# Juleszwanen/oscar_mpc_planner_mr_modification

Hardware: AMD Instinct MI355X
Metric: SQP solves/s (N=20, 8 obs, 8 guesses) at 1/2/4/8 MI355X; max |x−x_ref| (higher is better)
Workload: dtype f64

## Files before the change

__graft_entry__.py:

```python
import os
import sys

ROOT = os.path.dirname(os.path.abspath(__file__))
if ROOT not in sys.path:
    sys.path.insert(0, ROOT)


def build() -> None:
    from oscar_mpc_planner_mr_modification_amd import _build

    _build.build_lib()
    for cfg in ("C2", "C5", "C3", "JS"):
        _build.build_cpp(cfg)
    from oscar_mpc_planner_mr_modification_amd.layouts import tmpc_layout
    _build.build_instance(tmpc_layout(N=25, max_obstacles=3, name="G25"), os.path.join(_build.BUILD, "G25"))
    _build.build_stage_probe()
    sys.path.insert(0, os.path.join(ROOT, "oracle"))
    import oracle_py

    oracle_py.build()
    import oscar_mpc_planner_mr_modification_amd
    from oscar_mpc_planner_mr_modification_amd import native


def smoke() -> None:
    import numpy as np
    import torch

    sys.path.insert(0, os.path.join(ROOT, "oracle"))
    import oracle_py
    from oscar_mpc_planner_mr_modification_amd import native
    from oscar_mpc_planner_mr_modification_amd.layouts import config_layout
    from oscar_mpc_planner_mr_modification_amd.synthetic import make_batch

    assert torch.cuda.is_available(), "smoke() needs an MI355X"
    dev = torch.device("cuda:0")
    lay = config_layout("C2")
    b = make_batch(lay, 2, 8, seed=20251212)
    pr = native.problem_from_layout(lay)
    t = lambda a: torch.from_numpy(np.ascontiguousarray(a)).to(dev)
    out = native.solve_batch_device(pr, t(b.params), t(b.warm), t(b.xinit))
    torch.cuda.synchronize()
    ref = oracle_py.Oracle(lay).solve_batch(b.params, b.warm, b.xinit)
    exit_gpu = out["exit"].cpu().numpy()
    assert np.array_equal(exit_gpu, ref["status"]), (exit_gpu, ref["status"])
    ok = exit_gpu == 1
    assert ok.any()
    dx = np.abs(out["xtraj"].cpu().numpy()[ok] - ref["xtraj"][ok]).max()
    assert dx <= 1e-4, dx
    print(f"smoke ok: {len(exit_gpu)} solves, {int(ok.sum())} successful, max|x-x_ref| = {dx:.2e}")


if __name__ == "__main__":
    build()
    if len(sys.argv) > 1 and sys.argv[1] == "smoke":
        smoke()
```

oscar_mpc_planner_mr_modification_amd/_build.py:

```python
from __future__ import annotations

import os
import subprocess

PKG = os.path.dirname(os.path.abspath(__file__))
ROOT = os.path.dirname(PKG)
CSRC = os.path.join(PKG, "csrc")
INCLUDE = os.path.join(ROOT, "include")
LIB = os.path.join(PKG, "libmpcg.so")
ARCH = os.environ.get("MPCG_OFFLOAD_ARCH", "gfx950")

SOURCES = {"mpcg_kernels.hip": [], "mpcg_prepare.hip": ["-ffp-contract=off"],
           "mpcg_inst_tmpc20.hip": [], "mpcg_inst_tmpc30.hip": [], "mpcg_inst_shmpc.hip": [],
           "mpcg_inst_bicycle.hip": []}
HEADERS = ["mpcg_device.h", "mpcg_sqp.h", "mpcg_sqp_body.inc", "mpcg_prepare.h", "mpcg_bicycle.h", "mpcg_instance.h"]
FLEET_SOURCES = {"mpcg_fleet.hip": ["-ffp-contract=off"]}
FLEET_HEADERS = ["mpcg_fleet.h"]
PATH_SOURCES = {"mpcg_path.hip": ["-ffp-contract=off"]}
PATH_HEADERS = ["mpcg_path.h"]
GUIDANCE_SOURCES = {"mpcg_guidance.hip": ["-ffp-contract=off"]}
GUIDANCE_HEADERS = ["mpcg_guidance.h"]
ACTIVE_SOURCES = {"mpcg_active.hip": ["-ffp-contract=off"]}
ACTIVE_HEADERS = ["mpcg_active.h"]
HOST_SOURCES = ["host/mpcg_yaml.cpp", "host/mpcg_solver.cpp"]
HOST_HEADERS = ["mpc_planner_solver/mpcg_yaml.h", "mpc_planner_solver/mpcg_config.h", "mpc_planner_solver/state.h",
                "mpc_planner_solver/mpcg_solver_interface.h", "mpc_planner_solver/solver_interface.h"]
BUILD = os.path.join(PKG, "build")


def source_hash() -> str:
    import hashlib

    h = hashlib.sha256()
    for f in sorted(list(SOURCES) + HEADERS):
        h.update(f.encode())
        with open(os.path.join(CSRC, f), "rb") as fh:
            h.update(fh.read())
    with open(os.path.join(INCLUDE, "mpcg.h"), "rb") as fh:
        h.update(fh.read())
    h.update(repr((ARCH, sorted(SOURCES.items()))).encode())
    return h.hexdigest()


def _stale(target, deps):
    if not os.path.exists(target):
        return True
    t = os.path.getmtime(target)
    return any(os.path.getmtime(d) > t for d in deps)


def build_lib(force: bool = False, verbose: bool = False, extra_flags=(), out: str = LIB, sources=None) -> str:
    srcs = SOURCES if sources is None else {k: v for k, v in SOURCES.items() if k in sources}
    srcs = {**srcs, **FLEET_SOURCES, **PATH_SOURCES, **GUIDANCE_SOURCES, **ACTIVE_SOURCES}
    deps = [os.path.join(CSRC, s) for s in list(SOURCES) + HEADERS + list(FLEET_SOURCES) + FLEET_HEADERS +
            list(PATH_SOURCES) + PATH_HEADERS + list(GUIDANCE_SOURCES) + GUIDANCE_HEADERS +
            list(ACTIVE_SOURCES) + ACTIVE_HEADERS] + \
        [os.path.join(INCLUDE, h) for h in ("mpcg.h", "mpcg_fleet.h", "mpcg_path.h", "mpcg_guidance.h",
                                            "mpcg_active.h")] + [__file__]
    if not force and not _stale(out, deps):
        return out
    objdir = os.path.join(BUILD, "obj" + ("_" + "_".join(f.strip("-").replace("=", "") for f in extra_flags)
                                          if extra_flags else ""))
    os.makedirs(objdir, exist_ok=True)
    common = ["hipcc", f"--offload-arch={ARCH}", "-O3", "-std=c++17", "-fPIC", f"-I{INCLUDE}", f"-I{CSRC}"]
    objs, procs = [], []
    for src, flags in srcs.items():
        obj = os.path.join(objdir, src.replace(".hip", ".o"))
        cmd = common + list(flags) + list(extra_flags) + ["-c", os.path.join(CSRC, src), "-o", obj]
        if verbose:
            print(" ".join(cmd))
        procs.append(subprocess.Popen(cmd))
        objs.append(obj)
    for p in procs:
        if p.wait() != 0:
            raise subprocess.CalledProcessError(p.returncode, "hipcc")
    cmd = ["hipcc", f"--offload-arch={ARCH}", "-shared", "-fPIC", "-Wl,-soname,libmpcg.so", "-o", out + ".tmp"] + objs
    if verbose:
        print(" ".join(cmd))
    subprocess.run(cmd, check=True)
    os.replace(out + ".tmp", out)
    return out


def _hipcc_obj(src, obj, extra=()):
    cmd = ["hipcc", f"--offload-arch={ARCH}", "-O3", "-std=c++17", "-fPIC", f"-I{INCLUDE}", f"-I{CSRC}",
           *extra, "-c", src, "-o", obj]
    subprocess.run(cmd, check=True)
    return obj


def build_instance(layout, out_dir: str, force: bool = False) -> str:
    from . import codegen

    lib_mpcg = build_lib()
    os.makedirs(out_dir, exist_ok=True)
    src = os.path.join(out_dir, "mpcg_instance.hip")
    text = codegen.instance_source(layout)
    if not os.path.exists(src) or open(src).read() != text:
        with open(src, "w") as fh:
            fh.write(text)
    so = os.path.join(out_dir, f"libmpcg_inst_{layout.name}.so")
    deps = [src, lib_mpcg, os.path.join(INCLUDE, "mpcg.h")] + [os.path.join(CSRC, h) for h in HEADERS]
    if force or _stale(so, deps):
        obj = _hipcc_obj(src, os.path.join(out_dir, "mpcg_instance.o"))
        subprocess.run(["hipcc", f"--offload-arch={ARCH}", "-shared", "-fPIC", "-o", so + ".tmp", obj, f"-L{PKG}",
                        "-lmpcg", f"-Wl,-rpath,{PKG}"], check=True)
        os.replace(so + ".tmp", so)
    return so


def build_stage_probe(force: bool = False) -> str:
    src = os.path.join(ROOT, "tests", "cpp", "stage_probe.hip")
    out_dir = os.path.join(BUILD, "probe")
    so = os.path.join(out_dir, "libstage_probe.so")
    deps = [src, os.path.join(INCLUDE, "mpcg.h"), __file__] + [os.path.join(CSRC, h) for h in HEADERS]
    if force or _stale(so, deps):
        os.makedirs(out_dir, exist_ok=True)
        obj = _hipcc_obj(src, os.path.join(out_dir, "stage_probe.o"))
        subprocess.run(["hipcc", f"--offload-arch={ARCH}", "-shared", "-fPIC", "-o", so + ".tmp", obj], check=True)
        os.replace(so + ".tmp", so)
    return so


def build_cpp(config="C2", force: bool = False, verbose: bool = False) -> dict:
    from . import codegen
    from .layouts import config_layout

    lay = config_layout(config) if isinstance(config, str) else config
    lib_mpcg = build_lib()
    out = os.path.join(BUILD, lay.name)
    codegen.generate(lay, out)
    so = os.path.join(out, "libmpc_planner_solver.so")
    exe = os.path.join(out, "test_solver")
    srcs = [os.path.join(CSRC, s) for s in HOST_SOURCES] + [os.path.join(out, "mpc_planner_parameters.cpp")]
    inst = os.path.join(out, "mpcg_instance.hip")
    deps = srcs + [inst] + [os.path.join(INCLUDE, h) for h in HOST_HEADERS] + \
        [os.path.join(CSRC, h) for h in HEADERS] + [os.path.join(INCLUDE, "mpcg.h"), lib_mpcg, __file__]
    inc = [f"-I{os.path.join(out, 'include')}", f"-I{INCLUDE}"]
    if force or _stale(so, deps):
        objs = []
        for src in srcs:
            obj = os.path.join(out, os.path.basename(src).replace(".cpp", ".o"))
            cmd = ["g++", "-std=c++17", "-O2", "-fPIC", "-Wall", "-Wextra"] + inc + ["-c", src, "-o", obj]
            if verbose:
                print(" ".join(cmd))
            subprocess.run(cmd, check=True)
            objs.append(obj)
        objs.append(_hipcc_obj(inst, os.path.join(out, "mpcg_instance.o")))
        cmd = ["hipcc", f"--offload-arch={ARCH}", "-shared", "-fPIC"] + objs + \
              ["-o", so + ".tmp", f"-L{PKG}", "-lmpcg", f"-Wl,-rpath,{PKG}"]
        if verbose:
            print(" ".join(cmd))
        subprocess.run(cmd, check=True)
        os.replace(so + ".tmp", so)
    test_src = os.path.join(ROOT, "tests", "cpp", "test_solver.cpp")
    if os.path.exists(test_src) and (force or _stale(exe, [test_src, so])):
        cmd = ["g++", "-std=c++17", "-O2", "-Wall", "-Wextra"] + inc + [test_src, "-o", exe, f"-L{out}",
                                                                      "-lmpc_planner_solver", f"-L{PKG}", "-lmpcg",
                                                                      f"-Wl,-rpath,{out}:{PKG}"]
        if verbose:
            print(" ".join(cmd))
        subprocess.run(cmd, check=True)
    return {"dir": out, "lib": so, "test": exe}


if __name__ == "__main__":
    print(build_lib(force=True, verbose=True))
    print(build_cpp("C2", force=True, verbose=True))
```

oscar_mpc_planner_mr_modification_amd/csrc/mpcg_device.h:

```cpp
#pragma once
#include <hip/hip_runtime.h>

#include "mpcg.h"

namespace mpcg {

constexpr int NU = MPCG_NU;

__device__ __forceinline__ double frcp(double x) {
    double y = __builtin_amdgcn_rcp(x);
    double e = fma(-x, y, 1.0);
    y = fma(y, e, y);
    e = fma(-x, y, 1.0);
    return fma(y, e, y);
}

__device__ __forceinline__ double frsq(double x) {
    double y = __builtin_amdgcn_rsq(x);
    const double h = 0.5 * x;
    y = y * fma(-h * y, y, 1.5);
    return y * fma(-h * y, y, 1.5);
}

__device__ __forceinline__ double fsqrt_pos(double x) { return x * frsq(x); }
// ... 128 lines not shown
    const double wc = p[pr.i_w_contour], wl = p[pr.i_w_lag];
    double L = wa * a * a + ww * w * w + wv * (v - vref) * (v - vref);
    SplineJets J;
    spline_jets(pr, p, s, J);
    const double rsq = J.Dx[0] * J.Dx[0] + J.Dy[0] * J.Dy[0];
    const double ir = frsq(rsq);
    const double tx = J.Dx[0] * ir, ty = J.Dy[0] * ir;
    const double ex = x - J.Gx[0], ey = y - J.Gy[0];
    const double ec = ty * ex - tx * ey;
    const double el = tx * ex + ty * ey;
    L += wl * el * el + wc * ec * ec;
    double wcn = 0.0, dxp = 0.0, dyp = 0.0;
    if (pr.i_cons_w >= 0) {
        wcn = p[pr.i_cons_w];
        dxp = x - p[pr.i_prev_x];
        dyp = y - p[pr.i_prev_y];
        L += wcn * (dxp * dxp + dyp * dyp);
    }
    double wsl = 0.0, sl = 0.0;
    if constexpr (NX > 5) {
        wsl = p[pr.i_w_slack];
        sl = z[NU + 5];
        L += wsl * sl * sl;
    }
    if (!derivs) return L;
    const double r1 = tx * J.Dx[1] + ty * J.Dy[1];
    const double tx1 = (J.Dx[1] - tx * r1) * ir, ty1 = (J.Dy[1] - ty * r1) * ir;
    const double r2 = tx1 * J.Dx[1] + ty1 * J.Dy[1] + tx * J.Dx[2] + ty * J.Dy[2];
    const double tx2 = (J.Dx[2] - 2.0 * tx1 * r1 - tx * r2) * ir;
    const double ty2 = (J.Dy[2] - 2.0 * ty1 * r1 - ty * r2) * ir;
    const double Gx1 = J.Gx[1], Gy1 = J.Gy[1], Gx2 = J.Gx[2], Gy2 = J.Gy[2];
    const double dc[3] = {ty, -tx, ty1 * ex - tx1 * ey - ty * Gx1 + tx * Gy1};
    const double dl[3] = {tx, ty, tx1 * ex + ty1 * ey - tx * Gx1 - ty * Gy1};
    const double hc_s[3] = {ty1, -tx1, ty2 * ex - tx2 * ey - 2.0 * ty1 * Gx1 + 2.0 * tx1 * Gy1 - ty * Gx2 + tx * Gy2};
    const double hl_s[3] = {tx1, ty1, tx2 * ex + ty2 * ey - 2.0 * tx1 * Gx1 - 2.0 * ty1 * Gy1 - tx * Gx2 - ty * Gy2};
#pragma unroll
    for (int i = 0; i < NZ; ++i) {
        g[i] = 0.0;
#pragma unroll
        for (int j = 0; j < NZ; ++j) H[i][j] = 0.0;
    }
    g[0] = 2.0 * wa * a; H[0][0] = 2.0 * wa;
    g[1] = 2.0 * ww * w; H[1][1] = 2.0 * ww;
    g[5] = 2.0 * wv * (v - vref); H[5][5] = 2.0 * wv;
    constexpr int ids[3] = {2, 3, 6};
#pragma unroll
    for (int i = 0; i < 3; ++i) {
        g[ids[i]] += 2.0 * (wl * el * dl[i] + wc * ec * dc[i]);
#pragma unroll
        for (int j = 0; j < 3; ++j) {
            double hl = (i == 2) ? hl_s[j] : ((j == 2) ? hl_s[i] : 0.0);
            double hc = (i == 2) ? hc_s[j] : ((j == 2) ? hc_s[i] : 0.0);
            H[ids[i]][ids[j]] += 2.0 * (wl * (dl[i] * dl[j] + el * hl) + wc * (dc[i] * dc[j] + ec * hc));
        }
    }
    if (pr.i_cons_w >= 0) {
        g[2] += 2.0 * wcn * dxp; g[3] += 2.0 * wcn * dyp;
        H[2][2] += 2.0 * wcn; H[3][3] += 2.0 * wcn;
    }
    if constexpr (NX > 5) {
        g[NU + 5] = 2.0 * wsl * sl;
        H[NU + 5][NU + 5] = 2.0 * wsl;
    }
    return L;
}

__device__ __forceinline__ void erk_srow(const mpcg_problem& pr, double& sa, double& sv) {
    sa = 0.5 * pr.dt * pr.dt;
    sv = pr.dt;
}

template <int NX>
__device__ inline void erk_unicycle(const mpcg_problem& pr, const double z[NU + NX], const double* pi,
                                    double xn[NX], double F[NX][NU + NX], double H[NU + NX][NU + NX]) {
    constexpr int NZ = NU + NX;
    const double a = z[0], w = z[1], psi = z[4], v = z[5];
    const int ns = pr.rk_steps;
    const double h = pr.dt / ns;
    double sx = 0.0, sy = 0.0, ss = 0.0;
    double jx[4] = {0, 0, 0, 0}, jy[4] = {0, 0, 0, 0}, js[4] = {0, 0, 0, 0};
    double hq[4][4];
#pragma unroll
    for (int i = 0; i < 4; ++i)
#pragma unroll
        for (int j = 0; j < 4; ++j) hq[i][j] = 0.0;
    const double pix = pi ? pi[0] : 0.0, piy = pi ? pi[1] : 0.0;
    double cpsi, spsi;
    sincos(psi, &spsi, &cpsi);
    for (int st = 0; st < ns; ++st) {
#pragma unroll
        for (int q = 0; q < 4; ++q) {
            const double cq = (q == 0) ? 0.0 : ((q == 3) ? 1.0 : 0.5);
            const double bq = ((q == 0 || q == 3) ? 1.0 : 2.0) * h / 6.0;
            const double tau = (st + cq) * h;
            double sw, cw;
            sincos(tau * w, &sw, &cw);
            const double ce = cpsi * cw - spsi * sw;
            const double se = spsi * cw + cpsi * sw;
            const double ve = v + tau * a;
            sx += bq * ve * ce;
            sy += bq * ve * se;
            ss += bq * ve;
            const double dcx_p = -ve * se, dcx_v = ce;
            const double dcy_p = ve * ce, dcy_v = se;
            jx[0] += bq * dcx_v * tau; jx[1] += bq * dcx_p * tau; jx[2] += bq * dcx_p; jx[3] += bq * dcx_v;
            jy[0] += bq * dcy_v * tau; jy[1] += bq * dcy_p * tau; jy[2] += bq * dcy_p; jy[3] += bq * dcy_v;
            if (pi) {
                const double hpp = bq * (-pix * ve * ce - piy * ve * se);
                const double hpv = bq * (-pix * se + piy * ce);
                const double rp[4] = {0.0, tau, 1.0, 0.0};
                const double rv[4] = {tau, 0.0, 0.0, 1.0};
#pragma unroll
                for (int i = 0; i < 4; ++i)
#pragma unroll
                    for (int j = 0; j < 4; ++j)
                        hq[i][j] += hpp * rp[i] * rp[j] + hpv * (rp[i] * rv[j] + rv[i] * rp[j]);
            }
        }
    }
    erk_srow(pr, js[0], js[3]);
    const double T = pr.dt;
    xn[0] = z[2] + sx;
    xn[1] = z[3] + sy;
    xn[2] = psi + T * w;
    xn[3] = v + T * a;
    xn[4] = z[6] + ss;
#pragma unroll
    for (int i = 0; i < NX; ++i)
#pragma unroll
        for (int j = 0; j < NZ; ++j) F[i][j] = 0.0;
    constexpr int zi[4] = {0, 1, 4, 5};
#pragma unroll
    for (int j = 0; j < 4; ++j) {
        F[0][zi[j]] = jx[j];
        F[1][zi[j]] = jy[j];
        F[4][zi[j]] = js[j];
    }
    F[0][2] = 1.0; F[1][3] = 1.0; F[4][6] = 1.0;
    F[2][1] = T; F[2][4] = 1.0;
    F[3][0] = T; F[3][5] = 1.0;
#pragma unroll
    for (int i = 5; i < NX; ++i) {
        xn[i] = z[NU + i];
        F[i][NU + i] = 1.0;
    }
    if (pi) {
#pragma unroll
        for (int i = 0; i < 4; ++i)
#pragma unroll
            for (int j = 0; j < 4; ++j) H[zi[i]][zi[j]] += hq[i][j];
    }
}

template <int NZ, int NA = NZ>
__device__ inline void mirror(double A[NZ][NZ], double eps, double dia_extra = 0.0) {
    double V[NA][NA];
#pragma unroll
    for (int i = 0; i < NA; ++i)
#pragma unroll
        for (int j = 0; j < NA; ++j) {
            V[i][j] = (i == j) ? 1.0 : 0.0;
            if (j > i) A[i][j] = 0.5 * (A[i][j] + A[j][i]);
        }
    for (int sweep = 0; sweep < 50; ++sweep) {
        double off = 0.0, dia = 0.0;
#pragma unroll
        for (int i = 0; i < NA; ++i) {
            dia += A[i][i] * A[i][i];
            if (i == NA - 1) dia += dia_extra;
#pragma unroll
            for (int j = i + 1; j < NA; ++j) off += A[i][j] * A[i][j];
        }
        if (off <= 1e-32 * dia || off < 1e-300) break;
#pragma unroll
        for (int p = 0; p < NA - 1; ++p)
#pragma unroll
            for (int q = p + 1; q < NA; ++q) {
                const double apq = A[p][q];
                if (fabs(apq) >= 1e-300) {
                    const double theta = 0.5 * (A[q][q] - A[p][p]) * frcp(apq);
                    const double at = fabs(theta);
                    double t = at < 1e150 ? frcp(at + fsqrt_pos(fma(at, at, 1.0))) : 0.5 * frcp(at);
                    t = theta >= 0.0 ? t : -t;
                    const double c = frsq(fma(t, t, 1.0)), sn = t * c;
                    const double tau = sn * frcp(1.0 + c);
                    A[p][p] -= t * apq;
                    A[q][q] += t * apq;
                    A[p][q] = 0.0;
#pragma unroll
                    for (int r = 0; r < NA; ++r) {
                        if (r == p || r == q) continue;
                        double& arp = r < p ? A[r][p] : A[p][r];
                        double& arq = r < q ? A[r][q] : A[q][r];
                        const double g = arp, h = arq;
                        arp = g - sn * fma(g, tau, h);
                        arq = h + sn * fma(-h, tau, g);
                    }
#pragma unroll
                    for (int r = 0; r < NA; ++r) {
                        const double g = V[r][p], h = V[r][q];
                        V[r][p] = g - sn * fma(g, tau, h);
                        V[r][q] = h + sn * fma(-h, tau, g);
                    }
                }
            }
    }
    double d[NA];
#pragma unroll
    for (int i = 0; i < NA; ++i) {
        double di = A[i][i];
        d[i] = (di >= -eps && di <= eps) ? eps : fabs(di);
    }
#pragma unroll
    for (int i = 0; i < NA; ++i)
#pragma unroll
        for (int j = i; j < NA; ++j) {
            double acc = 0.0;
#pragma unroll
            for (int k = 0; k < NA; ++k) acc += V[i][k] * d[k] * V[j][k];
            A[i][j] = acc;
            A[j][i] = acc;
        }
}

}
```

oscar_mpc_planner_mr_modification_amd/csrc/mpcg_sqp.h:

```cpp
#pragma once
#include <hip/hip_runtime.h>

#include <type_traits>

#include "mpcg.h"
#include "mpcg_bicycle.h"
#include "mpcg_device.h"

namespace mpcg {

enum { AC_SUCCESS = 0, AC_NAN = 1, AC_MAXITER = 2, AC_MINSTEP = 3, AC_QP_FAILURE = 4 };

__host__ __device__ constexpr int imax(int a, int b) { return a > b ? a : b; }
__host__ __device__ constexpr int sym(int i, int j) { return i >= j ? i * (i + 1) / 2 + j : j * (j + 1) / 2 + i; }
__host__ __device__ constexpr int cpk(int n, int a, int c) { return c * n - c * (c - 1) / 2 + (a - c); }

__host__ __device__ constexpr int lds_b64_cycles(int s, int off, int parts) {
    int total = 0;
    for (int half = 0; half < 2; ++half) {
        int dw[64] = {};
        int n = 0;
        for (int l = 32 * half; l < 32 * half + 32; ++l) {
            const int a = 2 * (s * (l / parts) + off * (l % parts));
            for (int h = 0; h < 2; ++h) {
                bool seen = false;
                for (int i = 0; i < n; ++i) seen = seen || dw[i] == a + h;
                if (!seen) dw[n++] = a + h;
            }
        }
        int worst = 0;
        for (int b = 0; b < 64; ++b) {
            int c = 0;
            for (int i = 0; i < n; ++i) c += (dw[i] % 64) == b;
            worst = c > worst ? c : worst;
        }
        total += worst;
    }
    return total;
}
__host__ __device__ constexpr int lds_stride(int base, int off, int parts, int step, int maxpad) {
    int best = base, bc = lds_b64_cycles(base, off, parts);
    for (int s = base + step; s <= base + maxpad; s += step) {
        const int c = lds_b64_cycles(s, off, parts);
        if (c < bc) { bc = c; best = s; }
    }
    return best;
}

template <int N_, int NL_, int NE_, int NS_ = 0, int NX_ = 5, int MODEL_ = 0>
struct Cfg {
    static constexpr int N = N_, NL = NL_, NE = NE_, NS = NS_, MODEL = MODEL_;
    static constexpr int NU = MODEL_ == 1 ? 3 : 2;
    static constexpr int NX = NX_, NZ = NU + NX_;
    static_assert(MODEL_ == 1 ? NX == 6 : (NX == 5 || NX == 6), "unicycle (+ slack state) or bicycle");
    static constexpr int IX = NU, IY = NU + 1, IPSI = NU + 2;
    static constexpr bool HAS_SLACK = MODEL_ == 1 || NX > 5;
    static constexpr int ZSL = MODEL_ == 1 ? 2 : NU + 5;
    static constexpr int NLO = NU * (NU - 1) / 2, NLC = NU == 2 ? 4 : NLO + NU;
    __host__ __device__ static constexpr int lo_idx(int i, int j) { return i * (i - 1) / 2 + j; }
    static constexpr int NH = NL + NE + NS;
    static constexpr int NTRI = NZ * (NZ + 1) / 2;
    static constexpr int NPT = NX * (NX + 1) / 2;
    static constexpr int NPTP = (MODEL_ != 1 && (64 / (N_ + 1)) >= 3) ? NPT + (NPT & 1) : NPT;
    static constexpr int NB = (HAS_SLACK && NS > 0) ? 4 : 3;
    static constexpr int NBT = NB * (NB + 1) / 2;
    static constexpr int NDH = NZ + NBT + 1;
#ifndef MPCG_PARTS_BIKE
#define MPCG_PARTS_BIKE 2
#endif
    static constexpr int PARTS_MAX = (64 / (N + 1)) >= 3 ? 3 : 2;
    static constexpr int PARTS = MODEL_ == 1 ? (MPCG_PARTS_BIKE < PARTS_MAX ? MPCG_PARTS_BIKE : PARTS_MAX) : PARTS_MAX;
    static_assert((N + 1) * PARTS <= 64, "horizon too long for one wavefront");
    static_assert(NTRI <= 64, "stage block larger than a wavefront");
    static constexpr bool QUEUE = MODEL_ == 0 && PARTS_MAX == 3;
    static constexpr int BVS = (NZ + PARTS - 1) / PARTS;
    static constexpr int HS = (NH + PARTS - 1) / PARTS;
    static constexpr int SLOTS = 2 * BVS + HS;
#ifdef MPCG_STORE_IT_ANY
    static constexpr bool STORE_IT_ANY = true;
#else
    static constexpr bool STORE_IT_ANY = false;
#endif
    static constexpr bool STORE_IT = SLOTS <= (PARTS == 3 ? 13 : STORE_IT_ANY ? 12 : 0);
    static constexpr int NBOX = 2 * NU + 2 * NX;
    static constexpr bool LIN_PARAMS = NS > 0 || N >= 30;
    static constexpr int DGC = LIN_PARAMS ? 2 : 3;
    static constexpr int NHS = LIN_PARAMS ? (NE > 0 ? NE : 1) : NH;
    static constexpr bool RELOAD_PARAMS = NS > 0 || N >= 30;
    static constexpr int M_TOTAL = 2 * NU + (N - 1) * (NBOX + NH);
    __host__ __device__ static constexpr int blk(int v) {
        return (v >= IX && v <= IPSI) ? v - IX : ((NB == 4 && v == ZSL) ? 3 : -1);
    }
    __host__ __device__ static constexpr int bvar(int b) { return b < 3 ? IX + b : ZSL; }
    static constexpr bool COMPACT = MODEL_ == 1;
    static constexpr bool FCONST = MODEL_ == 0 && N_ >= 30;
    static constexpr int NFR = COMPACT ? 4 : (FCONST ? 2 : NX), NFC = COMPACT ? NZ - 1 : NZ;
    static constexpr int NHP = COMPACT ? (NZ - 1) * NZ / 2 + 1 : NTRI;
    static constexpr bool CHAIN_SPLIT = !COMPACT;
    static constexpr bool PAIR_WANTED = FCONST && NE_ <= 8;
    static constexpr bool PAIR_CHAINS = PAIR_WANTED && CHAIN_SPLIT && (N_ + 1) / 2 * NX_ * NX_ <= (N_ + 1) * NDH &&
                                        (N_ + 1) / 2 * NX_ <= 128;
    static constexpr bool FAC_FLAT = !COMPACT;
    static constexpr bool REC_FLAT = CHAIN_SPLIT && PARTS == 3;
#ifndef MPCG_RES_CARRY
#define MPCG_RES_CARRY 1
#endif
    static constexpr bool RES_CARRY = MPCG_RES_CARRY > 0 && MODEL_ == 0 && PARTS == 3 && NX_ == 5;
    static constexpr int QPM_ROWS = 2 * SLOTS * 64;
    static constexpr int QPM = QPM_ROWS + (N + 1) * NZ + N * NX;
    __host__ __device__ static constexpr double slack_coef(int hh) { return (NB == 4 && hh >= NL + NE) ? -1.0 : 0.0; }
};

template <class C, bool LEAN = C::COMPACT, bool GFH = false, int PAD = 0>
struct Lds {
    static constexpr int N = C::N, NX = C::NX, NZ = C::NZ;
    static constexpr int DGS =
        PAD ? lds_stride(C::NHS * C::DGC, C::DGC, C::PARTS, C::DGC % 2 == 0 ? 2 : 1, 3) : C::NHS * C::DGC;
    static constexpr int HDS = PAD ? lds_stride(C::NHS, 1, C::PARTS, 1, 3) : C::NHS;
    static constexpr int PS = PAD == 0   ? C::NPTP
                              : PAD == 2 ? lds_stride(C::NPT + (C::NPT & 1), 0, C::PARTS, 2, 4)
                                         : lds_stride(C::NPTP, 0, C::PARTS, C::NPTP == C::NPT ? 1 : 2, 4);
    double z[N + 1][NZ];
    double H[GFH ? 1 : N + 1][C::NHP];
    double g[N + 1][NZ];
    double F[GFH ? 1 : N][C::NFR][C::NFC];
    double Fst[GFH && !C::COMPACT ? C::NFR : 1][C::NFC];
    double Hst[GFH && !C::COMPACT ? C::NHP : 1];
    double b[N][NX];
    double dH[N + 1][C::NDH];
    double q[N + 1][NZ];
    double dz[N + 1][NZ];
    double ddz[N + 1][NZ];
    double pi_nlp[N][NX];
    double piq[N][NX];
    double pin[LEAN ? 1 : N][NX];
    double rdyn[LEAN ? 1 : N][NX];
    alignas(16) double P[N + 1][PS];
    double Lc[N][C::NLC];
    double Y[N][C::NU][NX];
    double bx[N + 1][NZ];
    double Dg[N][DGS];
    double hd[N][HDS];
    double disc[C::LIN_PARAMS ? N : 1][4];
    double Msc[128];
    double xinit[NX];
    int flag;
};

constexpr size_t LDS_QUARTER = 160 * 1024 / 4;
template <class C>
__host__ __device__ constexpr bool lds_lean() {
    return C::COMPACT || (sizeof(Lds<C, false>) > LDS_QUARTER && sizeof(Lds<C, true>) <= LDS_QUARTER);
}
template <class C>
__host__ __device__ constexpr bool lds_gfh() {
    return sizeof(Lds<C, lds_lean<C>(), false>) > LDS_QUARTER && sizeof(Lds<C, lds_lean<C>(), true>) <= LDS_QUARTER;
}
template <class C>
__host__ __device__ constexpr int lds_pad() {
    constexpr bool P_ALIGN = !C::COMPACT;
    return P_ALIGN && sizeof(Lds<C, lds_lean<C>(), lds_gfh<C>(), 2>) <= LDS_QUARTER ? 2
           : sizeof(Lds<C, lds_lean<C>(), lds_gfh<C>(), 1>) <= LDS_QUARTER         ? 1
                                                                                   : 0;
}
template <class C>
using LdsOf = Lds<C, lds_lean<C>(), lds_gfh<C>(), lds_pad<C>()>;
template <class C>
__host__ __device__ constexpr size_t gfh_doubles() {
    return lds_gfh<C>() ? (size_t)C::N * C::NFR * C::NFC + (size_t)(C::N + 1) * C::NHP : 0;
}
template <class C>
__host__ __device__ constexpr size_t itref_doubles() {
    return 2 * (size_t)(C::N + 1) * C::NZ + (size_t)C::N * C::NX;
}
template <class C>
__host__ __device__ constexpr size_t ws_doubles() {
    return gfh_doubles<C>() + itref_doubles<C>();
}

#ifdef MPCG_STAMPS
#define MPCG_NSTAMP 24
#define STAMP_DECL unsigned long long st_acc_[MPCG_NSTAMP] = {}, st_t0_ = 0, st_l_ = 0;
#define STAMP_BEGIN() do { __syncthreads(); st_t0_ = __builtin_amdgcn_s_memtime(); st_l_ = st_t0_; } while (0)
#define STAMP_END(i) do { __syncthreads(); st_acc_[i] += __builtin_amdgcn_s_memtime() - st_t0_; } while (0)
#define STAMP_LAP(i) do { const unsigned long long t_ = __builtin_amdgcn_s_memtime(); st_acc_[i] += t_ - st_l_; st_l_ = t_; } while (0)
#define STAMP_STORE(ptr, sol) \
    do { if ((ptr) && threadIdx.x == 0) for (int i_ = 0; i_ < MPCG_NSTAMP; ++i_) (ptr)[(size_t)(sol) * MPCG_NSTAMP + i_] = st_acc_[i_]; } while (0)
#elif defined(MPCG_MARKERS)
#define STAMP_DECL
#define STAMP_BEGIN() asm volatile("; @@begin")
#define STAMP_END(i) asm volatile("; @@end " #i)
#define STAMP_LAP(i) asm volatile("; @@lap " #i)
#define STAMP_STORE(ptr, sol) do {} while (0)
#else
#define STAMP_DECL
#define STAMP_BEGIN() do {} while (0)
#define STAMP_END(i) do {} while (0)
#define STAMP_LAP(i) do {} while (0)
#define STAMP_STORE(ptr, sol) do {} while (0)
#endif

__device__ __forceinline__ void wave_sync() { __asm__ volatile("" ::: "memory"); }

typedef __attribute__((address_space(3))) double lds_double;
__device__ __forceinline__ unsigned sel_lanes(unsigned long long mask, unsigned off, unsigned on) {
    unsigned r;
    asm volatile("v_cndmask_b32_e64 %0, %1, %2, %3" : "=v"(r) : "v"(off), "v"(on), "s"(mask));
    return r;
}
__device__ __forceinline__ unsigned lds_addr(double* p) { return (unsigned)(size_t)(lds_double*)p; }
__device__ __forceinline__ void lds_store(unsigned a, double v) { *(lds_double*)(size_t)a = v; }
__device__ __forceinline__ double readlane_d(double v, int lane) {
    const int lo = __builtin_amdgcn_readlane(__double2loint(v), lane);
    const int hi = __builtin_amdgcn_readlane(__double2hiint(v), lane);
    return __hiloint2double(hi, lo);
}
template <int CTRL, int ROW_MASK = 0xF>
__device__ __forceinline__ double dpp_d(double v) {
    const int lo = __builtin_amdgcn_update_dpp(__double2loint(v), __double2loint(v), CTRL, ROW_MASK, 0xF, false);
    const int hi = __builtin_amdgcn_update_dpp(__double2hiint(v), __double2hiint(v), CTRL, ROW_MASK, 0xF, false);
    return __hiloint2double(hi, lo);
}
__device__ __forceinline__ double lane_down(double v, int p) {
    double w = dpp_d<0x130>(v);
    if (p == 2) w = dpp_d<0x130>(w);
    return w;
}
__device__ __forceinline__ double wave_max(double v) {
    v = fmax(v, dpp_d<0xB1>(v));
    v = fmax(v, dpp_d<0x4E>(v));
    v = fmax(v, dpp_d<0x141>(v));
    v = fmax(v, dpp_d<0x140>(v));
    v = fmax(v, dpp_d<0x142, 0xA>(v));
    v = fmax(v, dpp_d<0x143, 0xC>(v));
    return readlane_d(v, 63);
}
__device__ __forceinline__ double wave_sum(double v) {
    v += dpp_d<0xB1>(v);
    v += dpp_d<0x4E>(v);
    v += dpp_d<0x141>(v);
    v += dpp_d<0x140>(v);
    v += dpp_d<0x142, 0xA>(v);
    v += dpp_d<0x143, 0xC>(v);
    return readlane_d(v, 63);
}


template <int n>
__device__ __forceinline__ double chain_dot(double h, const double* G, const double* v) {
    double a = h;
#pragma unroll
    for (int j = 0; j < n; ++j) a += G[j] * v[j];
    return a;
}

template <class C>
__device__ __forceinline__ double dh_at(const double* dh, int i, int j) {
    double v = (i == j) ? dh[i] : 0.0;
    const int a = C::blk(i), c = C::blk(j);
    if (a >= 0 && c >= 0) v += dh[C::NZ + (a >= c ? cpk(C::NB, a, c) : cpk(C::NB, c, a))];
// ... 159 lines not shown
```

oscar_mpc_planner_mr_modification_amd/csrc/mpcg_sqp_body.inc:

```
    constexpr int N = C::N, PARTS = C::PARTS, NX = C::NX, NZ = C::NZ, NB = C::NB, NBT = C::NBT;
    constexpr int NU = C::NU;
    constexpr int ZS = C::ZSL;
    constexpr int X0 = C::IX, X1 = C::IY, X2 = C::IPSI;
    constexpr bool LEAN = lds_lean<C>();
    constexpr bool GFH = lds_gfh<C>();
    constexpr bool RES_SPLIT = !C::COMPACT && 2 * NB <= NZ && PARTS == 3 && NX == 5;
    constexpr int DRS = (NX + PARTS - 1) / PARTS;
    static_assert(!(RES_SPLIT && LEAN), "the split passes read the dynamics multipliers from S.pin");
    constexpr bool RES_CARRY = C::RES_CARRY && RES_SPLIT && !LEAN;
    constexpr bool CFLAG = !LEAN && !C::HAS_SLACK;
    __shared__ LdsOf<C> S;
    if (sol >= batch) return;
    if (blockDim.x != 64) {
        if (threadIdx.x == 0) io.exit_code[sol] = -1;
        return;
    }
#ifdef MPCG_LDS_POISON
    for (int e = threadIdx.x; e < (int)(sizeof(S) / 8); e += 64) ((double*)&S)[e] = __builtin_nan("");
    wave_sync();
#endif
    int lane_ = threadIdx.x;
    if constexpr (C::QUEUE) __asm__ volatile("" : "+v"(lane_));
    const int lane = lane_;
    const int k = lane / PARTS;
// ... 73 lines not shown
            return S.hd[k][hh - C::NL];
        } else {
            return S.hd[k][hh];
        }
    };
    double srow_a = 0.0, srow_v = 0.0;
    if constexpr (C::FCONST) erk_srow(pr, srow_a, srow_v);
    auto FatB = [&](const double (*Fk)[C::NFC], int m, int j) -> double {
        if constexpr (C::FCONST) {
            if (m == 2) return j == 1 ? pr.dt : (j == 4 ? 1.0 : 0.0);
            if (m == 3) return j == 0 ? pr.dt : (j == 5 ? 1.0 : 0.0);
            if (m == 4) return j == 0 ? srow_a : (j == 5 ? srow_v : (j == 6 ? 1.0 : 0.0));
            if (m >= 5) return j == NU + m ? 1.0 : 0.0;
            return Fk[m][j];
        } else if constexpr (C::COMPACT) {
            if (m == 3) return j == bike::ZV ? 1.0 : (j == bike::ZA ? pr.dt : 0.0);
            if (m == 4) return j == bike::ZDELTA ? 1.0 : (j == bike::ZW ? pr.dt : 0.0);
            if (j == ZS) return 0.0;
            return Fk[m < 3 ? m : 3][j < ZS ? j : j - 1];
        } else {
            return Fk[m][j];
        }
    };
    auto HatB = [&](const double* Hk, int i, int j) -> double {
        if constexpr (C::COMPACT) {
            if (i == ZS || j == ZS) return (i == j) ? Hk[C::NHP - 1] : 0.0;
            return Hk[sym(i < ZS ? i : i - 1, j < ZS ? j : j - 1)];
        } else {
            return Hk[sym(i, j)];
        }
    };
    auto Fat = [&](int kq, int m, int j) -> double { return FatB(Fb(kq), m, j); };
    auto Hat = [&](int kq, int i, int j) -> double { return HatB(Hb(kq), i, j); };
    auto rdyn_at = [&](int kq, int i) -> double {
        double a = S.b[kq][i] - S.dz[kq + 1][NU + i];
#pragma unroll
        for (int j = 0; j < NZ; ++j) a += Fat(kq, i, j) * S.dz[kq][j];
        return a;
    };
    auto stepped = [](double x, double a, double dx) -> double { return x + a * dx; };
    Rows<C> R;
#pragma unroll
    for (int r = 0; r < HS; ++r)
        R.nlam[r] = (lam_in && LR.h_on(r)) ? lam_in[(size_t)k * LAMS + NX + LR.hrow(r)] : 0.0;

    const double* w = io.warm + (size_t)sol * (N + 1) * NZ;
    for (int e = lane; e < (N + 1) * NZ; e += 64) (&S.z[0][0])[e] = w[e];
    for (int e = lane; e < N * NX; e += 64)
        (&S.pi_nlp[0][0])[e] = lam_in ? lam_in[(size_t)(e / NX) * LAMS + e % NX] : 0.0;
    if (lane < NX) S.xinit[lane] = io.xinit[(size_t)sol * NX + lane];
    for (int e = lane; e <= N; e += 64) S.dH[e][C::NDH - 1] = 0.0;
    const bool qp_warm = FULL && pr.qp_warm_start == 2;
    const bool sqp_mode = FULL && pr.nlp_solver == MPCG_NLP_SQP;
    bool have_qp = false;
    if (FULL && io.qp_in && !isnan(io.qp_in[(size_t)sol * C::QPM])) {
        const double* q = io.qp_in + (size_t)sol * C::QPM;
#pragma unroll
        for (int sl = 0; sl < C::SLOTS; ++sl) {
            R.t[sl] = q[(2 * sl) * 64 + lane];
            R.l[sl] = q[(2 * sl + 1) * 64 + lane];
        }
        for (int e = lane; e < (N + 1) * NZ; e += 64) (&S.dz[0][0])[e] = q[C::QPM_ROWS + e];
        for (int e = lane; e < N * NX; e += 64) (&S.piq[0][0])[e] = q[C::QPM_ROWS + (N + 1) * NZ + e];
        have_qp = true;
    }
    wave_sync();
    if (lane < NU) S.z[N][lane] = 0.0;
    wave_sync();

    constexpr bool PH = PROF == PROF_HPIPM, PRB = PROF == PROF_ROBUST;
    const bool p_move = PH ? true : PRB ? false : pr.qp_init_move != 0;
    const bool p_cond = PH ? true : PRB ? false : pr.qp_cond_pred_corr != 0;
    const int p_itref = PH ? 2 : PRB ? 0 : pr.qp_itref_corr_max;
    const bool p_sclip = PH ? false : PRB ? true : pr.qp_sigma_clip != 0;
    const bool p_maxit_first = PH ? true : PRB ? false : pr.qp_maxit_first != 0;
    const bool p_pzero = PH ? true : PRB ? false : pr.qp_pivot_zero != 0;
    const double mu_max = PH ? __builtin_inf() : pr.qp_mu_max > 0.0 ? pr.qp_mu_max : __builtin_inf(), tmin = pr.qp_t_min;
    const bool itref_on = p_itref > 0;
    int acados_status = AC_SUCCESS, qp_status = AC_SUCCESS, sqp_iter = 0, qp_total = 0, n_maxit = 0;
    double res_eq = 0.0;
    double nlp_stat = 0.0, nlp_ineq = 0.0, nlp_comp = 0.0;
    bool nlp_nonfinite = false;

    for (int it = 0; sqp_mode || it < pr.sqp_iters; ++it) {
        if constexpr (C::RELOAD_PARAMS) asm volatile("" : "+v"(pk));
        STAMP_BEGIN();
        {
            double zk[NZ];
#pragma unroll
            for (int i = 0; i < NZ; ++i) zk[i] = S.z[ks][i];
            double hb6[6] = {0, 0, 0, 0, 0, 0};
            if (k >= 1 && k < N) h_rows<C>(pr, pk, zk, LR, R.nlam, hb6, (double (*)[C::DGC])S.Dg[k], S.hd[k], S.disc[C::LIN_PARAMS ? k : 0]);
            STAMP_LAP(10);
            {
                double acc[6];
#pragma unroll
                for (int i = 0; i < 6; ++i) acc[i] = hb6[i];
#pragma unroll
                for (int p = 1; p < PARTS; ++p)
#pragma unroll
                    for (int i = 0; i < 6; ++i) acc[i] += lane_down(hb6[i], p);
#pragma unroll
                for (int i = 0; i < 6; ++i) hb6[i] = acc[i];
            }
            double resl = 0.0;
            double H[NZ][NZ];
            if (stage_lane && k < N) {
                double g[NZ], xn[NX], pi[NX];
#pragma unroll
                for (int i = 0; i < NX; ++i) pi[i] = S.pi_nlp[k][i];
                if constexpr (C::MODEL == 1) {
                    double* const Hd = Hb(k);
                    bike::discrete(pr, pk, zk, pi, xn, Fb(k), Hd);
                    STAMP_LAP(12);
                    bike::stage_cost(pr, pk, k, zk, g, H, true);
                    STAMP_LAP(11);
#pragma unroll
                    for (int i = 0; i < NZ; ++i)
#pragma unroll
                        for (int j = 0; j < NZ; ++j)
                            if (i != ZS && j != ZS) H[i][j] += Hd[sym(i < ZS ? i : i - 1, j < ZS ? j : j - 1)];
#pragma unroll
                    for (int i = 0; i < NX; ++i) {
                        const double bi = xn[i] - S.z[k + 1][NU + i];
                        S.b[k][i] = bi;
                        resl = fmax(resl, fabs(bi));
                    }
                } else {
                    double F[NX][NZ];
                    stage_cost<NX>(pr, pk, zk, g, H, true);
                    STAMP_LAP(11);
                    erk_unicycle<NX>(pr, zk, pi, xn, F, H);
                    STAMP_LAP(12);
#pragma unroll
                    for (int i = 0; i < NX; ++i) {
                        const double bi = xn[i] - S.z[k + 1][NU + i];
                        S.b[k][i] = bi;
                        resl = fmax(resl, fabs(bi));
                        if (i < C::NFR) {
#pragma unroll
                            for (int j = 0; j < NZ; ++j) Fb(k)[i][j] = F[i][j];
                        }
                    }
                }
#pragma unroll
                for (int i = 0; i < NZ; ++i) S.g[k][i] = g[i];
                H[X0][X0] += hb6[0]; H[X0][X1] += hb6[1]; H[X1][X0] += hb6[1];
                H[X0][X2] += hb6[2]; H[X2][X0] += hb6[2];
                H[X1][X1] += hb6[3]; H[X1][X2] += hb6[4]; H[X2][X1] += hb6[4];
                H[X2][X2] += hb6[5];
                STAMP_LAP(13);
                if constexpr (C::MODEL == 0 && NZ == 8) {
                    const double hs = H[NZ - 1][NZ - 1];
                    mirror<NZ, NZ - 1>(H, pr.reg_eps, hs * hs);
                    H[NZ - 1][NZ - 1] = (hs >= -pr.reg_eps && hs <= pr.reg_eps) ? pr.reg_eps : fabs(hs);
                } else if constexpr (C::MODEL == 1) {
                    double Hp[NZ][NZ];
#pragma unroll
                    for (int i = 0; i < NZ; ++i)
#pragma unroll
                        for (int j = 0; j < NZ; ++j) {
                            const int pi2 = i == NZ - 1 ? ZS : (i < ZS ? i : i + 1);
                            const int pj2 = j == NZ - 1 ? ZS : (j < ZS ? j : j + 1);
                            Hp[i][j] = H[pi2][pj2];
                        }
                    const double hs = Hp[NZ - 1][NZ - 1];
                    mirror<NZ, NZ - 1>(Hp, pr.reg_eps, hs * hs);
                    Hp[NZ - 1][NZ - 1] = (hs >= -pr.reg_eps && hs <= pr.reg_eps) ? pr.reg_eps : fabs(hs);
#pragma unroll
                    for (int i = 0; i < NZ; ++i)
#pragma unroll
                        for (int j = 0; j < NZ; ++j) {
                            const int pi2 = i == NZ - 1 ? ZS : (i < ZS ? i : i + 1);
                            const int pj2 = j == NZ - 1 ? ZS : (j < ZS ? j : j + 1);
                            H[pi2][pj2] = Hp[i][j];
                        }
                } else {
                    mirror<NZ>(H, pr.reg_eps);
                }
                STAMP_LAP(14);
                if constexpr (C::COMPACT) {
#pragma unroll
                    for (int i = 0; i < NZ; ++i)
#pragma unroll
                        for (int j = 0; j <= i; ++j)
                            if (i != ZS && j != ZS) Hb(k)[sym(i < ZS ? i : i - 1, j < ZS ? j : j - 1)] = H[i][j];
                    Hb(k)[C::NHP - 1] = H[ZS][ZS];
                } else {
#pragma unroll
                    for (int i = 0; i < NZ; ++i)
#pragma unroll
                        for (int j = 0; j <= i; ++j) Hb(k)[sym(i, j)] = H[i][j];
                }
            } else if (stage_lane && k == N) {
#pragma unroll
                for (int i = 0; i < NZ; ++i) S.g[N][i] = 0.0;
#pragma unroll
                for (int e = 0; e < C::NHP; ++e) Hb(N)[e] = 0.0;
#pragma unroll
                for (int i = NU; i < NZ; ++i) {
                    if constexpr (C::COMPACT) Hb(N)[sym(i - 1, i - 1)] = pr.reg_eps;
                    else Hb(N)[sym(i, i)] = pr.reg_eps;
                }
            }
            res_eq = wave_max(resl);
            if (lane < NX) S.dz[0][NU + lane] = S.xinit[lane] - S.z[0][NU + lane];
        }
        if constexpr (GFH) __builtin_amdgcn_fence(__ATOMIC_ACQ_REL, "workgroup");
        wave_sync();
        STAMP_END(0);

        STAMP_BEGIN();
        if (FULL && (io.stats || sqp_mode)) {
            double rh[NB];
#pragma unroll
            for (int i = 0; i < NB; ++i) rh[i] = 0.0;
            double vin = 0.0, vcp = 0.0, vst = 0.0;
            double chk = 0.0;
#pragma unroll
            for (int j = 0; j < BVS; ++j) {
                double lb = 0.0;
                if (LR.box_on(j)) {
                    const double zv = S.z[k][LR.var(j)];
                    const double gl = zv - LR.lo_at(j), gh = LR.hi_at(j) - zv;
                    const double ll = have_qp ? R.l[2 * j] : 0.0, lh = have_qp ? R.l[2 * j + 1] : 0.0;
                    chk += 0.0 * (zv + ll + lh);
                    vin = fmax(vin, -gl);
                    vin = fmax(vin, -gh);
                    vcp = fmax(vcp, fabs(ll * gl));
                    vcp = fmax(vcp, fabs(lh * gh));
                    lb = lh - ll;
                }
                if (k <= N && LR.var(j) < NZ) S.bx[k][LR.var(j)] = lb;
            }
#pragma unroll
            for (int r = 0; r < HS; ++r) {
                if (!LR.h_on(r)) continue;
                const int hh = LR.hrow(r);
                double a, bq, c;
                rowg(hh, a, bq, c);
                const double gap = rowgap(hh);
                const double lam = have_qp ? R.l[HB + r] : R.nlam[r];
                rh[0] += a * lam; rh[1] += bq * lam; rh[2] += c * lam;
                if constexpr (NB == 4) rh[3] += C::slack_coef(hh) * lam;
                vin = fmax(vin, -gap);
                vcp = fmax(vcp, fabs(lam * gap));
                chk += 0.0 * (gap + lam);
            }
            double acc[NB];
#pragma unroll
            for (int i = 0; i < NB; ++i) acc[i] = rh[i];
#pragma unroll
            for (int p = 1; p < PARTS; ++p)
#pragma unroll
                for (int i = 0; i < NB; ++i) acc[i] += lane_down(rh[i], p);
            wave_sync();
            if (stage_lane) {
                double r[NZ];
#pragma unroll
                for (int i = 0; i < NZ; ++i) r[i] = S.g[k][i] + S.bx[k][i];
#pragma unroll
                for (int i = 0; i < NB; ++i) r[C::bvar(i)] += acc[i];
                if (k < N) {
#pragma unroll
                    for (int m = 0; m < NX; ++m) {
                        const double pm = S.pi_nlp[k][m];
#pragma unroll
                        for (int i = 0; i < NZ; ++i) r[i] += Fat(k, m, i) * pm;
                    }
                }
                if (k > 0) {
#pragma unroll
                    for (int i = 0; i < NX; ++i) r[NU + i] -= S.pi_nlp[k - 1][i];
                }
#pragma unroll
                for (int i = 0; i < NZ; ++i) {
                    const bool free_var = (k == N) ? (i >= NU) : ((k == 0) ? (i < NU) : true);
                    if (free_var) vst = fmax(vst, fabs(r[i]));
                    chk += 0.0 * r[i];
                }
                if (k < N) {
#pragma unroll
                    for (int i = 0; i < NX; ++i) chk += 0.0 * S.b[k][i];
                }
            }
            nlp_stat = wave_max(vst);
            nlp_ineq = wave_max(vin);
            nlp_comp = wave_max(vcp);
            nlp_nonfinite = !(wave_sum(chk) == 0.0);
            wave_sync();
        }
        if (sqp_mode) {
            if (nlp_nonfinite) {
                acados_status = AC_NAN;
                break;
            }
            if (nlp_stat < pr.nlp_tol && res_eq < pr.nlp_tol && nlp_ineq < pr.nlp_tol && nlp_comp < pr.nlp_tol) {
                acados_status = AC_SUCCESS;
                break;
            }
            if (it >= pr.nlp_max_iter) {
                acados_status = AC_MAXITER;
                break;
            }
        }
        const bool warm_now = qp_warm && have_qp && ((sqp_mode && it > 0) || pr.qp_warm_first);
        bool hcold = false;
        if (warm_now) {
            const double thr = pr.qp_ws_thr;
#pragma unroll
            for (int sl = 0; sl < C::SLOTS; ++sl) {
                if (R.t[sl] < thr) R.t[sl] = thr;
                if (R.l[sl] < thr) R.l[sl] = thr;
                R.pr[sl] = 0.0;
            }
        } else {
        if (stage_lane) {
#pragma unroll
            for (int i = 0; i < NZ; ++i)
                if (!(k == 0 && i >= NU)) S.dz[k][i] = 0.0;
            if (k < N) {
#pragma unroll
                for (int i = 0; i < NX; ++i) S.piq[k][i] = 0.0;
            }
        }
        {
            const double thr0 = pr.qp_thr0, mu0 = pr.qp_mu0;
            const bool mv = p_move;
            auto cold = [&](int s, double gap) {
// ... 1672 lines not shown
```

Baseline: 556,500.

## Exploit block structure of stage Hessian in Jacobi eigen-regularisation

Adds a block-diagonal variant of the Jacobi eigenvalue mirror routine that skips rotations, updates and reconstruction terms coupling the two independent index blocks of the unicycle's 7x7 Hessian. A wave-wide ballot checks that the cross-block entries are exactly zero and finite on every lane, and falls back to the full routine otherwise. The intent is to cut the per-stage Jacobi sweep cost. In exchange it adds a check and a branch, and the sweep order and convergence test change, which could shift numerics slightly. It is enabled by default for PARTS==3, NX==5 model-0 configs, and a probe build target is added.

```diff
diff --git a/__graft_entry__.py b/__graft_entry__.py
--- a/__graft_entry__.py
+++ b/__graft_entry__.py
@@ -15,6 +15,7 @@
     from oscar_mpc_planner_mr_modification_amd.layouts import tmpc_layout
     _build.build_instance(tmpc_layout(N=25, max_obstacles=3, name="G25"), os.path.join(_build.BUILD, "G25"))
     _build.build_stage_probe()
+    _build.build_mirror_probe()
     sys.path.insert(0, os.path.join(ROOT, "oracle"))
     import oracle_py
 
diff --git a/oscar_mpc_planner_mr_modification_amd/_build.py b/oscar_mpc_planner_mr_modification_amd/_build.py
--- a/oscar_mpc_planner_mr_modification_amd/_build.py
+++ b/oscar_mpc_planner_mr_modification_amd/_build.py
@@ -122,6 +122,19 @@
     return so
 
 
+def build_mirror_probe(force: bool = False) -> str:
+    src = os.path.join(ROOT, "tests", "cpp", "mirror_probe.hip")
+    out_dir = os.path.join(BUILD, "probe")
+    so = os.path.join(out_dir, "libmirror_probe.so")
+    deps = [src, os.path.join(INCLUDE, "mpcg.h"), __file__, os.path.join(CSRC, "mpcg_device.h")]
+    if force or _stale(so, deps):
+        os.makedirs(out_dir, exist_ok=True)
+        obj = _hipcc_obj(src, os.path.join(out_dir, "mirror_probe.o"))
+        subprocess.run(["hipcc", f"--offload-arch={ARCH}", "-shared", "-fPIC", "-o", so + ".tmp", obj], check=True)
+        os.replace(so + ".tmp", so)
+    return so
+
+
 def build_cpp(config="C2", force: bool = False, verbose: bool = False) -> dict:
     from . import codegen
     from .layouts import config_layout
diff --git a/oscar_mpc_planner_mr_modification_amd/csrc/mpcg_device.h b/oscar_mpc_planner_mr_modification_amd/csrc/mpcg_device.h
--- a/oscar_mpc_planner_mr_modification_amd/csrc/mpcg_device.h
+++ b/oscar_mpc_planner_mr_modification_amd/csrc/mpcg_device.h
@@ -304,13 +304,17 @@
     }
 }
 
-template <int NZ, int NA = NZ>
+__host__ __device__ constexpr int mirror_blk(int i) { return (i == 2 || i == 3 || i == 6) ? 1 : 0; }
+template <int NZ, int NA = NZ, bool BLOCKS = false>
 __device__ inline void mirror(double A[NZ][NZ], double eps, double dia_extra = 0.0) {
+    static_assert(!BLOCKS || NA == 7, "the block form is the unicycle's 7 x 7 block");
+    constexpr auto in = [](int i, int j) { return !BLOCKS || mirror_blk(i) == mirror_blk(j); };
     double V[NA][NA];
 #pragma unroll
     for (int i = 0; i < NA; ++i)
 #pragma unroll
         for (int j = 0; j < NA; ++j) {
+            if (!in(i, j)) continue;
             V[i][j] = (i == j) ? 1.0 : 0.0;
             if (j > i) A[i][j] = 0.5 * (A[i][j] + A[j][i]);
         }
@@ -321,13 +325,15 @@
             dia += A[i][i] * A[i][i];
             if (i == NA - 1) dia += dia_extra;
 #pragma unroll
-            for (int j = i + 1; j < NA; ++j) off += A[i][j] * A[i][j];
+            for (int j = i + 1; j < NA; ++j)
+                if (in(i, j)) off += A[i][j] * A[i][j];
         }
         if (off <= 1e-32 * dia || off < 1e-300) break;
 #pragma unroll
         for (int p = 0; p < NA - 1; ++p)
 #pragma unroll
             for (int q = p + 1; q < NA; ++q) {
+                if (!in(p, q)) continue;
                 const double apq = A[p][q];
                 if (fabs(apq) >= 1e-300) {
                     const double theta = 0.5 * (A[q][q] - A[p][p]) * frcp(apq);
@@ -341,7 +347,7 @@
                     A[p][q] = 0.0;
 #pragma unroll
                     for (int r = 0; r < NA; ++r) {
-                        if (r == p || r == q) continue;
+                        if (r == p || r == q || !in(r, p)) continue;
                         double& arp = r < p ? A[r][p] : A[p][r];
                         double& arq = r < q ? A[r][q] : A[q][r];
                         const double g = arp, h = arq;
@@ -350,6 +356,7 @@
                     }
 #pragma unroll
                     for (int r = 0; r < NA; ++r) {
+                        if (!in(r, p)) continue;
                         const double g = V[r][p], h = V[r][q];
                         V[r][p] = g - sn * fma(g, tau, h);
                         V[r][q] = h + sn * fma(-h, tau, g);
@@ -369,10 +376,32 @@
         for (int j = i; j < NA; ++j) {
             double acc = 0.0;
 #pragma unroll
-            for (int k = 0; k < NA; ++k) acc += V[i][k] * d[k] * V[j][k];
+            for (int k = 0; k < NA; ++k)
+                if (in(i, j) && in(i, k)) acc += V[i][k] * d[k] * V[j][k];
             A[i][j] = acc;
             A[j][i] = acc;
         }
 }
 
-}
+template <int NZ>
+__device__ inline bool mirror_blocks_ok(const double A[NZ][NZ]) {
+    bool ok = true;
+#pragma unroll
+    for (int i = 0; i < 7; ++i)
+#pragma unroll
+        for (int j = i; j < 7; ++j) {
+            if (mirror_blk(i) != mirror_blk(j)) ok &= (A[i][j] == 0.0) & (A[j][i] == 0.0);
+            else ok &= __builtin_isfinite(i == j ? A[i][i] : 0.5 * (A[i][j] + A[j][i]));
+        }
+    return ok;
+}
+
+template <int NZ, int NA = NZ>
+__device__ inline bool mirror_stage(double A[NZ][NZ], double eps, double dia_extra = 0.0) {
+    const bool blocks = __builtin_amdgcn_ballot_w64(!mirror_blocks_ok<NZ>(A)) == 0;
+    if (blocks) mirror<NZ, NA, true>(A, eps, dia_extra);
+    else mirror<NZ, NA>(A, eps, dia_extra);
+    return blocks;
+}
+
+}
diff --git a/oscar_mpc_planner_mr_modification_amd/csrc/mpcg_sqp.h b/oscar_mpc_planner_mr_modification_amd/csrc/mpcg_sqp.h
--- a/oscar_mpc_planner_mr_modification_amd/csrc/mpcg_sqp.h
+++ b/oscar_mpc_planner_mr_modification_amd/csrc/mpcg_sqp.h
@@ -106,6 +106,11 @@
 #define MPCG_RES_CARRY 1
 #endif
     static constexpr bool RES_CARRY = MPCG_RES_CARRY > 0 && MODEL_ == 0 && PARTS == 3 && NX_ == 5;
+#ifndef MPCG_MIRROR_BLOCKS
+#define MPCG_MIRROR_BLOCKS 1
+#endif
+    static constexpr bool MIRROR_BLOCKS =
+        MODEL_ == 0 && (MPCG_MIRROR_BLOCKS >= 2 || (MPCG_MIRROR_BLOCKS == 1 && PARTS == 3 && NX_ == 5));
     static constexpr int QPM_ROWS = 2 * SLOTS * 64;
     static constexpr int QPM = QPM_ROWS + (N + 1) * NZ + N * NX;
     __host__ __device__ static constexpr double slack_coef(int hh) { return (NB == 4 && hh >= NL + NE) ? -1.0 : 0.0; }
diff --git a/oscar_mpc_planner_mr_modification_amd/csrc/mpcg_sqp_body.inc b/oscar_mpc_planner_mr_modification_amd/csrc/mpcg_sqp_body.inc
--- a/oscar_mpc_planner_mr_modification_amd/csrc/mpcg_sqp_body.inc
+++ b/oscar_mpc_planner_mr_modification_amd/csrc/mpcg_sqp_body.inc
@@ -249,7 +249,8 @@
                 STAMP_LAP(13);
                 if constexpr (C::MODEL == 0 && NZ == 8) {
                     const double hs = H[NZ - 1][NZ - 1];
-                    mirror<NZ, NZ - 1>(H, pr.reg_eps, hs * hs);
+                    if constexpr (C::MIRROR_BLOCKS) mirror_stage<NZ, NZ - 1>(H, pr.reg_eps, hs * hs);
+                    else mirror<NZ, NZ - 1>(H, pr.reg_eps, hs * hs);
                     H[NZ - 1][NZ - 1] = (hs >= -pr.reg_eps && hs <= pr.reg_eps) ? pr.reg_eps : fabs(hs);
                 } else if constexpr (C::MODEL == 1) {
                     double Hp[NZ][NZ];
@@ -272,6 +273,8 @@
                             const int pj2 = j == NZ - 1 ? ZS : (j < ZS ? j : j + 1);
                             H[pi2][pj2] = Hp[i][j];
                         }
+                } else if constexpr (C::MIRROR_BLOCKS) {
+                    mirror_stage<NZ>(H, pr.reg_eps);
                 } else {
                     mirror<NZ>(H, pr.reg_eps);
                 }
```

After: 572,600 (median of 6 runs). 1.03x the previous value.
